# vribeiro1/artspeech

Hardware: AMD Instinct MI355X
Metric: articulator-frames/sec (fwd+bwd) (higher is better)
Workload: dtype f32

## Files before the change

### artspeech_amd/csrc/gru.hip

```cpp
#include <cstdlib>

#include <type_traits>

#include <hip/hip_ext.h>

#include "as_common.h"
#include "gemm_internal.h"

namespace {

typedef float f32x2 __attribute__((ext_vector_type(2)));

template <int LPU>
__device__ __forceinline__ float unit_sum(float v) {
    v += __int_as_float(__builtin_amdgcn_update_dpp(0, __float_as_int(v), 0xB1, 0xF, 0xF, true));
    if (LPU == 4) v += __int_as_float(__builtin_amdgcn_update_dpp(0, __float_as_int(v), 0x4E, 0xF, 0xF, true));
    return v;
}

constexpr int AHEAD = 2;

template <int H, int LPU, bool TRAIN, bool TOK>
__global__ __launch_bounds__(LPU * H) void gru_fwd_kernel(const float* __restrict__ gi, const int64_t* __restrict__ tokens,
                                                          long tok_stride, const float* __restrict__ w_hh,
                                                          const float* __restrict__ b_hh, const int* __restrict__ lengths,
                                                          int T, float* __restrict__ y, float* __restrict__ gates, int nd, int V) {
    constexpr int CW = 4 * LPU;
    constexpr int NC = H / CW;
    constexpr int NT = LPU * H;
    __shared__ __attribute__((aligned(16))) float hbuf[3][H];
    extern __shared__ int tok_s[];
    const int b = blockIdx.x, dir = blockIdx.y;
    const int tid = threadIdx.x, j = tid / LPU, q = tid % LPU;
    const int len = lengths[b];

    f32x2 w[3][NC * 2];
    {
        const float* wd = w_hh + (long)dir * 3 * H * H;
#pragma unroll
        for (int g = 0; g < 3; ++g)
#pragma unroll
            for (int c = 0; c < NC; ++c) {
                const float4 v = *reinterpret_cast<const float4*>(wd + (long)(g * H + j) * H + CW * c + 4 * q);
                w[g][2 * c] = f32x2{v.x, v.y};
                w[g][2 * c + 1] = f32x2{v.z, v.w};
            }
    }
    const float bq_r = b_hh[dir * 3 * H + j] * (1.0f / LPU), bq_z = b_hh[dir * 3 * H + H + j] * (1.0f / LPU),
                bq_n = b_hh[dir * 3 * H + 2 * H + j] * (1.0f / LPU);

    for (long i = (long)len * H + tid; i < (long)T * H; i += NT)
        y[((long)b * T + i / H) * nd * H + dir * H + (i % H)] = 0.f;
    if (tid < H) hbuf[0][tid] = 0.f;
    if (TOK)
        for (int t = tid; t < len; t += NT) {
            const int64_t v = tokens[(long)b * tok_stride + t];
            tok_s[t] = (int)(V > 0 ? min(max(v, (int64_t)0), (int64_t)V - 1) : v) * (nd * 3 * H * 4);
        }
    __syncthreads();
    if (len <= 0) return;

    const int t0 = dir ? len - 1 : 0;
    const int dt = dir ? -1 : 1;
    const unsigned ys = (unsigned)nd * H * 4u, gs = (unsigned)nd * 4u * H * 4u, is = (unsigned)nd * 3u * H * 4u;
    const unsigned yo = (unsigned)(dir * H + j) * 4u;
    const unsigned go = (unsigned)(dir * 4 * H + j + (LPU == 4 ? q * H : q * H)) * 4u;
    const unsigned io = (unsigned)(dir * 3 * H + j) * 4u;
    const char* gi_c = reinterpret_cast<const char*>(gi);
    char* y_c = reinterpret_cast<char*>(y);
    char* g_c = reinterpret_cast<char*>(gates);
    const int m0 = q == 0 ? -1 : 0, m1 = q == 1 ? -1 : 0, m2 = q == 2 ? -1 : 0, m3 = q == 3 ? -1 : 0;

    float h = 0.f;
    struct Gi { float r, z, n; };
    auto load_step = [&](int u) {
        const int uc = u < len ? u : len - 1;
        const int tu = t0 + uc * dt;
        const unsigned ro = (TOK ? (unsigned)tok_s[tu] : (unsigned)(b * T + tu) * is) + io;
        const float* p = reinterpret_cast<const float*>(gi_c + ro);
        return Gi{p[0], p[H], p[2 * H]};
    };
    auto step = [&](auto curc, int s, const Gi& ci, Gi& fill) {
        const int cur = curc, nxt = (cur + 1) % 3;
        const unsigned fr = (unsigned)(b * T + t0 + s * dt);
        fill = load_step(s + AHEAD);
        const float4* hp = reinterpret_cast<const float4*>(hbuf[cur]);
        f32x2 ar = {bq_r, 0.f}, az = {bq_z, 0.f}, an = {bq_n, 0.f};
#pragma unroll
        for (int c0 = 0; c0 < NC; c0 += 8) {
            float4 hv[8];
#pragma unroll
            for (int u = 0; u < 8; ++u)
                if (c0 + u < NC) hv[u] = hp[LPU * (c0 + u) + q];
            __builtin_amdgcn_sched_barrier(0);
#pragma unroll
            for (int u = 0; u < 8; ++u)
                if (c0 + u < NC) {
                    const int c = c0 + u;
                    const f32x2 lo = {hv[u].x, hv[u].y}, hi = {hv[u].z, hv[u].w};
                    ar = __builtin_elementwise_fma(w[0][2 * c], lo, ar);
                    az = __builtin_elementwise_fma(w[1][2 * c], lo, az);
                    an = __builtin_elementwise_fma(w[2][2 * c], lo, an);
                    ar = __builtin_elementwise_fma(w[0][2 * c + 1], hi, ar);
                    az = __builtin_elementwise_fma(w[1][2 * c + 1], hi, az);
                    an = __builtin_elementwise_fma(w[2][2 * c + 1], hi, an);
                }
        }
        const float sr = unit_sum<LPU>(ar.x + ar.y), sz = unit_sum<LPU>(az.x + az.y), sn = unit_sum<LPU>(an.x + an.y);
        float r, z;
        if constexpr (LPU == 4) {
            const float pre = __int_as_float((__float_as_int(ci.r + sr) & m0) | (__float_as_int(ci.z + sz) & ~m0));
            const float sg = as_sigmoid(pre);
            r = __int_as_float(__builtin_amdgcn_update_dpp(0, __float_as_int(sg), 0x00, 0xF, 0xF, true));
            z = __int_as_float(__builtin_amdgcn_update_dpp(0, __float_as_int(sg), 0x55, 0xF, 0xF, true));
        } else {
            r = as_sigmoid(ci.r + sr);
            z = as_sigmoid(ci.z + sz);
        }
        const float hn = sn;
        const float n = as_tanh(ci.n + r * hn);
        const float hnew = (1.f - z) * n + z * h;
        h = hnew;
        hbuf[nxt][j] = hnew;
        *reinterpret_cast<float*>(y_c + (fr * ys + yo)) = hnew;
        if (TRAIN) {
            float* gp = reinterpret_cast<float*>(g_c + (fr * gs + go));
            if (LPU == 4) {
                const int m01 = m0 | m1;
                const int t1 = (__float_as_int(r) & m0) | (__float_as_int(z) & ~m0);
                const int t2 = (__float_as_int(n) & m2) | (__float_as_int(hn) & ~m2);
                gp[0] = __int_as_float((t1 & m01) | (t2 & ~m01));
            } else {
                const int ga = (__float_as_int(r) & m0) | (__float_as_int(z) & m1);
                const int gc = (__float_as_int(n) & m0) | (__float_as_int(hn) & m1);
                gp[0] = __int_as_float(ga);
                gp[2 * H] = __int_as_float(gc);
            }
        }
        __syncthreads();
    };
    constexpr std::integral_constant<int, 0> c0{};
    constexpr std::integral_constant<int, 1> c1{};
    constexpr std::integral_constant<int, 2> c2{};
    Gi a = load_step(0), bq = load_step(1), c;
    int s = 0;
    for (; s + 2 < len; s += 3) {
        step(c0, s, a, c);
        step(c1, s + 1, bq, a);
        step(c2, s + 2, c, bq);
    }
    if (s < len) step(c0, s, a, c);
    if (s + 1 < len) step(c1, s + 1, bq, a);
}

template <int H, bool TOK, int ND = 2>
__global__ __launch_bounds__(4 * H) void gru_bwd_row_kernel(const float* __restrict__ dy, const float* __restrict__ y,
                                                            const float* __restrict__ gates, const float* __restrict__ w_hh,
                                                            const int* __restrict__ lengths, int T, float* __restrict__ dgi,
                                                            float* __restrict__ dgh, unsigned long long* __restrict__ dbg,
                                                            const int64_t* __restrict__ tokens, long tok_stride, int V,
                                                            float* __restrict__ part) {
    constexpr int NT = 4 * H;
    extern __shared__ float tab[];
    constexpr int VL = 3 * H / 16;
    unsigned long long t_start = 0, r_start = 0;
    if (dbg != nullptr && threadIdx.x == 0) {
        t_start = __builtin_amdgcn_s_memtime();
        r_start = __builtin_amdgcn_s_memrealtime();
    }
    constexpr int VW = VL % 4 == 0 ? 4 : 2;
    constexpr int NCH = VL / VW;
    __shared__ __attribute__((aligned(16))) float gbuf[3][3 * H];
    const int b = blockIdx.x, dir = blockIdx.y;
    const int tid = threadIdx.x, row = tid >> 4, r = tid & 15;
    const int k0 = row * 4, k = k0 + (r & 3), pl = r >> 2;
    const int len = lengths[b];

    f32x2 wt[4][VL / 2];
    {
        const float* wd = w_hh + (long)dir * 3 * H * H;
#pragma unroll
        for (int c = 0; c < NCH; ++c)
#pragma unroll
            for (int pp = 0; pp < VW / 2; ++pp) {
                const int i = (c * 16 + r) * VW + 2 * pp;
                const float4 lo = *reinterpret_cast<const float4*>(wd + (long)i * H + k0);
                const float4 hi = *reinterpret_cast<const float4*>(wd + (long)(i + 1) * H + k0);
                auto pick = [](const float4& v, int u) { return u == 0 ? v.x : u == 1 ? v.y : u == 2 ? v.z : v.w; };
#pragma unroll
                for (int sl = 0; sl < 4; ++sl) wt[sl][c * (VW / 2) + pp] = f32x2{pick(lo, (sl + (r & 3)) & 3), pick(hi, (sl + (r & 3)) & 3)};
            }
    }
    for (long i = (long)len * 3 * H + tid; i < (long)T * 3 * H; i += NT) {
        const long t = i / (3 * H), c = i % (3 * H);
        const long o = (((long)b * T + t) * ND + dir) * 3 * H + c;
        if constexpr (!TOK) dgi[o] = 0.f;
        dgh[o] = 0.f;
    }
    float* part_wg = nullptr;
    if constexpr (TOK) {
        for (int i = tid; i < V * 3 * H; i += NT) tab[i] = 0.f;
        int* toff = reinterpret_cast<int*>(tab + (long)V * 3 * H + NT);
        for (int t = tid; t < len; t += NT) toff[t] = (int)min(max(tokens[(long)b * tok_stride + t], (int64_t)0), (int64_t)V - 1) * (3 * H);
        part_wg = part + (long)b * V * 6 * H + (long)dir * 3 * H;
        if (len <= 0) {
            for (int i = tid; i < V * 3 * H; i += NT) part_wg[(long)(i / (3 * H)) * 6 * H + i % (3 * H)] = 0.f;
            return;
        }
    } else {
        if (len <= 0) return;
    }

    const int t0 = dir ? 0 : len - 1;
    const int dt = dir ? 1 : -1;
    const char* g_c = reinterpret_cast<const char*>(gates);
    const char* y_c = reinterpret_cast<const char*>(y);
    const char* dy_c = reinterpret_cast<const char*>(dy);
    char* dgi_c = reinterpret_cast<char*>(dgi);
    char* dgh_c = reinterpret_cast<char*>(dgh);
    const unsigned gto = (unsigned)(dir * 4 * H + k) * 4u;
    const unsigned yo = (unsigned)(dir * H + k) * 4u;
    const int sel = pl < 2 ? pl : 2;
    const unsigned dgo = (unsigned)(dir * 3 * H + sel * H + k) * 4u;
    struct In { float r, z, n, hn, hprev, dyv; bool has_prev; };
    auto load = [&](long fr, bool has_prev) {
        In v;
        const unsigned f = (unsigned)fr;
        const float* gp = reinterpret_cast<const float*>(g_c + (f * (ND * 4u * H * 4u) + gto));
        v.r = gp[0]; v.z = gp[H]; v.n = gp[2 * H]; v.hn = gp[3 * H];
        v.hprev = *reinterpret_cast<const float*>(y_c + ((f + (unsigned)(has_prev ? dt : 0)) * (ND * H * 4u) + yo));
        v.has_prev = has_prev;
        v.dyv = *reinterpret_cast<const float*>(dy_c + (f * (ND * H * 4u) + yo));
        return v;
    };
    auto dpp_add = [](float acc, float v, auto ctrl) {
        return acc + __int_as_float(__builtin_amdgcn_update_dpp(0, __float_as_int(v), decltype(ctrl)::value, 0xF, 0xF, true));
    };
    const long fbase = (long)b * T + t0;
    float dh = 0.f;
    const int tmask = pl < 3 ? -1 : 0;
    float* tabk = pl < 3 ? tab + sel * H + k : tab + (long)V * 3 * H + tid;
    const int* toff = reinterpret_cast<const int*>(tab + (long)V * 3 * H + NT);
    int toff_cur = 0;
    if constexpr (TOK) {
        __syncthreads();
        toff_cur = toff[t0];
    }
    auto load_step = [&](int u) {
        const int uc = u < len ? u : len - 1;
        return load(fbase + (long)uc * dt, uc + 1 < len);
    };
    auto step = [&](auto bulk, auto curc, int s, const In& ci, In& fill) {
        constexpr bool BULK = decltype(bulk)::value;
        const int cur = curc;
        const long fr = fbase + (long)s * dt;
        if constexpr (BULK) fill = load(fbase + (long)(s + AHEAD) * dt, true);
        else fill = load_step(s + AHEAD);

        const float rg = ci.r, z = ci.z, n = ci.n, hn = ci.hn;
        const float omz = 1.f - z;
        const float c_n = omz * (1.f - n * n);
        const float c_hn = c_n * rg;
        const float c_r = c_hn * hn * (1.f - rg);
        const float c_z = (((BULK || ci.has_prev) ? ci.hprev : 0.f) - n) * z * omz;
        const float c_rz = pl == 0 ? c_r : c_z;
        const float c_vi = pl >= 2 ? c_n : c_rz;
        const float c_vh = pl >= 2 ? c_hn : c_rz;
        const float dht = dh + ci.dyv;
        const float vi = dht * c_vi;
        const float vh = dht * c_vh;
        gbuf[cur][sel * H + k] = vh;
        const unsigned dfo = (unsigned)fr * (ND * 3u * H * 4u) + dgo;
        if constexpr (!TOK) *reinterpret_cast<float*>(dgi_c + dfo) = vi;
        *reinterpret_cast<float*>(dgh_c + dfo) = vh;
        __syncthreads();

        f32x2 a[4] = {{0.f, 0.f}, {0.f, 0.f}, {0.f, 0.f}, {0.f, 0.f}};
        if constexpr (VW == 4) {
            const float4* gq = reinterpret_cast<const float4*>(gbuf[cur]);
            float4 gv[NCH];
#pragma unroll
            for (int c = 0; c < NCH; ++c) gv[c] = gq[c * 16 + r];
            float* tw = nullptr;
            float told = 0.f;
            int toff_nxt = 0;
            if constexpr (TOK) {
                tw = tabk + (toff_cur & tmask);
                told = *tw;
                toff_nxt = toff[t0 + (s + 1 < len ? s + 1 : s) * dt];
            }
            __builtin_amdgcn_sched_barrier(0);
#pragma unroll
            for (int c = 0; c < NCH; ++c) {
                const f32x2 lo = {gv[c].x, gv[c].y}, hi = {gv[c].z, gv[c].w};
#pragma unroll
                for (int kk = 0; kk < 4; ++kk) {
                    a[kk] = __builtin_elementwise_fma(wt[kk][2 * c], lo, a[kk]);
                    a[kk] = __builtin_elementwise_fma(wt[kk][2 * c + 1], hi, a[kk]);
                }
            }
            if constexpr (TOK) {
                __builtin_amdgcn_sched_barrier(0);
                *tw = told + vi;
                toff_cur = toff_nxt;
            }
        } else {
            const float2* gq = reinterpret_cast<const float2*>(gbuf[cur]);
            float2 gv[NCH];
#pragma unroll
            for (int c = 0; c < NCH; ++c) gv[c] = gq[c * 16 + r];
            __builtin_amdgcn_sched_barrier(0);
#pragma unroll
            for (int c = 0; c < NCH; ++c) {
                const f32x2 g2 = {gv[c].x, gv[c].y};
#pragma unroll
                for (int kk = 0; kk < 4; ++kk) a[kk] = __builtin_elementwise_fma(wt[kk][c], g2, a[kk]);
            }
            if constexpr (TOK) {
                tabk[toff_cur & tmask] += vi;
                toff_cur = toff[t0 + (s + 1 < len ? s + 1 : s) * dt];
            }
        }
        float acc = a[0].x + a[0].y;
        acc = dpp_add(acc, a[3].x + a[3].y, std::integral_constant<int, 0x39>{});
        acc = dpp_add(acc, a[2].x + a[2].y, std::integral_constant<int, 0x4E>{});
        acc = dpp_add(acc, a[1].x + a[1].y, std::integral_constant<int, 0x93>{});
        acc = dpp_add(acc, acc, std::integral_constant<int, 0x124>{});
        acc = dpp_add(acc, acc, std::integral_constant<int, 0x128>{});
        dh = dht * z + acc;
    };
    constexpr std::integral_constant<int, 0> c0{};
    constexpr std::integral_constant<int, 1> c1{};
    constexpr std::integral_constant<int, 2> c2{};
    In a = load_step(0), bq = load_step(1), c;
    int s = 0;
    constexpr std::true_type yes{};
    constexpr std::false_type no{};
    for (; s + 5 < len; s += 3) {
        step(yes, c0, s, a, c);
        step(yes, c1, s + 1, bq, a);
        step(yes, c2, s + 2, c, bq);
    }
    for (; s + 2 < len; s += 3) {
        step(no, c0, s, a, c);
        step(no, c1, s + 1, bq, a);
        step(no, c2, s + 2, c, bq);
    }
    if (s < len) step(no, c0, s, a, c);
    if (s + 1 < len) step(no, c1, s + 1, bq, a);
    if constexpr (TOK) {
        __syncthreads();
        for (int i = tid; i < V * 3 * H; i += NT) part_wg[(long)(i / (3 * H)) * 6 * H + i % (3 * H)] = tab[i];
    }
    if (dbg != nullptr && threadIdx.x == 0) {
        unsigned long long* d = dbg + 4L * (blockIdx.y * gridDim.x + blockIdx.x);
        d[0] = __builtin_amdgcn_s_memtime() - t_start;
        d[1] = __builtin_amdgcn_s_memrealtime() - r_start;
        d[2] = (unsigned long long)len;
        d[3] = r_start;
    }
}


constexpr int GEN_THREADS = 1024;

template <bool TRAIN, bool TOK>
__global__ __launch_bounds__(GEN_THREADS) void gru_fwd_generic_kernel(const float* __restrict__ gi, const int64_t* __restrict__ tokens,
                                                                     long tok_stride, const float* __restrict__ w_hh,
                                                                     const float* __restrict__ b_hh, const int* __restrict__ lengths,
                                                                     int T, int H, float* __restrict__ y, float* __restrict__ gates,
                                                                     int nd, int V) {
    extern __shared__ __attribute__((aligned(16))) float gsm[];
    const int b = blockIdx.x, dir = blockIdx.y, tid = threadIdx.x;
    const int q = tid & 3;
    const int len = lengths[b];
    for (long i = (long)len * H + tid; i < (long)T * H; i += GEN_THREADS)
        y[((long)b * T + i / H) * nd * H + dir * H + (i % H)] = 0.f;
    for (int j = tid; j < 2 * H; j += GEN_THREADS) gsm[j] = 0.f;
    __syncthreads();
    if (len <= 0) return;
    const float* wd = w_hh + (long)dir * 3 * H * H;
    const float* bd = b_hh + (long)dir * 3 * H;
    const int nch = H >> 2;
    for (int s = 0; s < len; ++s) {
        const int t = dir ? len - 1 - s : s;
        const long frame = (long)b * T + t;
        const float* hc = gsm + (s & 1) * H;
        float* hn_ = gsm + ((s & 1) ^ 1) * H;
        const float* gr;
        if (TOK) {
            int64_t v = tokens[(long)b * tok_stride + t];
            if (V > 0) v = v < 0 ? 0 : (v >= V ? V - 1 : v);
            gr = gi + (v * nd + dir) * 3L * H;
        } else {
            gr = gi + (frame * nd + dir) * 3L * H;
        }
        for (int j = tid >> 2; j < H; j += GEN_THREADS / 4) {
            const float4* wr = reinterpret_cast<const float4*>(wd + (long)j * H);
            const float4* wz = reinterpret_cast<const float4*>(wd + (long)(H + j) * H);
            const float4* wn = reinterpret_cast<const float4*>(wd + (long)(2 * H + j) * H);
            const float4* h4 = reinterpret_cast<const float4*>(hc);
            float sr = 0.f, sz = 0.f, sn = 0.f;
            for (int c0 = q; c0 < nch; c0 += 16) {
                float4 a[4], c[4], e[4], hv[4];
#pragma unroll
                for (int u = 0; u < 4; ++u) {
                    const int cc = c0 + 4 * u;
                    const int ci = cc < nch ? cc : nch - 1;
                    a[u] = wr[ci]; c[u] = wz[ci]; e[u] = wn[ci];
                    hv[u] = h4[ci];
                    if (cc >= nch) hv[u] = make_float4(0.f, 0.f, 0.f, 0.f);
                }
#pragma unroll
                for (int u = 0; u < 4; ++u) {
                    sr += a[u].x * hv[u].x + a[u].y * hv[u].y + a[u].z * hv[u].z + a[u].w * hv[u].w;
                    sz += c[u].x * hv[u].x + c[u].y * hv[u].y + c[u].z * hv[u].z + c[u].w * hv[u].w;
                    sn += e[u].x * hv[u].x + e[u].y * hv[u].y + e[u].z * hv[u].z + e[u].w * hv[u].w;
                }
            }
            sr = unit_sum<4>(sr) + bd[j];
            sz = unit_sum<4>(sz) + bd[H + j];
            sn = unit_sum<4>(sn) + bd[2 * H + j];
            const float r = as_sigmoid(gr[j] + sr);
            const float z = as_sigmoid(gr[H + j] + sz);
            const float n = as_tanh(gr[2 * H + j] + r * sn);
            const float hnew = (1.f - z) * n + z * hc[j];
            if (q == 0) {
                hn_[j] = hnew;
                y[(frame * nd + dir) * H + j] = hnew;
                if (TRAIN) {
                    float* gp = gates + (frame * nd + dir) * 4L * H + j;
                    gp[0] = r; gp[H] = z; gp[2 * H] = n; gp[3 * H] = sn;
                }
            }
        }
        __syncthreads();
    }
}

__global__ __launch_bounds__(GEN_THREADS) void gru_bwd_generic_kernel(const float* __restrict__ dy, const float* __restrict__ y,
                                                                     const float* __restrict__ gates, const float* __restrict__ w_hh,
                                                                     const int* __restrict__ lengths, int T, int H,
                                                                     float* __restrict__ dgi, float* __restrict__ dgh, int nd) {
    extern __shared__ __attribute__((aligned(16))) float gsm[];
    float* gb = gsm;
    float* dhb = gsm + 3 * H;
    float* dhz = gsm + 4 * H;
    float* part = gsm + 5 * H;
    const int b = blockIdx.x, dir = blockIdx.y, tid = threadIdx.x;
    const int len = lengths[b];
    for (long i = (long)len * 3 * H + tid; i < (long)T * 3 * H; i += GEN_THREADS) {
        const long t = i / (3 * H), c = i % (3 * H);
        const long o = (((long)b * T + t) * nd + dir) * 3 * H + c;
        dgi[o] = 0.f;
        dgh[o] = 0.f;
    }
    for (int j = tid; j < H; j += GEN_THREADS) dhb[j] = 0.f;
    __syncthreads();
    if (len <= 0) return;
    const float* wd = w_hh + (long)dir * 3 * H * H;
    const int dt = dir ? 1 : -1;
    const int kq = tid >> 8, kl = tid & 255;
    for (int s = 0; s < len; ++s) {
        const int t = dir ? s : len - 1 - s;
        const long frame = (long)b * T + t;
        const bool has_prev = s + 1 < len;
        for (int j = tid; j < H; j += GEN_THREADS) {
            const float* gp = gates + (frame * nd + dir) * 4L * H + j;
            const float r = gp[0], z = gp[H], n = gp[2 * H], hn = gp[3 * H];
            const float hprev = has_prev ? y[((frame + dt) * nd + dir) * H + j] : 0.f;
            const float dht = dhb[j] + dy[(frame * nd + dir) * H + j];
            const float dn = dht * (1.f - z);
            const float dz = dht * (hprev - n);
            const float dnt = dn * (1.f - n * n);
            const float g_r = dnt * hn * r * (1.f - r);
            const float g_z = dz * z * (1.f - z);
            const float g_hn = dnt * r;
            float* di = dgi + (frame * nd + dir) * 3L * H + j;
            float* dh = dgh + (frame * nd + dir) * 3L * H + j;
            di[0] = g_r; di[H] = g_z; di[2 * H] = dnt;
            dh[0] = g_r; dh[H] = g_z; dh[2 * H] = g_hn;
            gb[j] = g_r; gb[H + j] = g_z; gb[2 * H + j] = g_hn;
            dhz[j] = dht * z;
        }
        __syncthreads();
        for (int k0 = 0; k0 < H; k0 += 256) {
            const int k = k0 + kl;
            const int kc = k < H ? k : H - 1;
            float acc = 0.f;
            for (int i0 = kq; i0 < 3 * H; i0 += 32) {
                float wv[8], gv[8];
#pragma unroll
                for (int u = 0; u < 8; ++u) {
                    const int i = i0 + 4 * u;
                    const int ic = i < 3 * H ? i : 3 * H - 1;
                    wv[u] = wd[(long)ic * H + kc];
                    gv[u] = i < 3 * H ? gb[ic] : 0.f;
                }
#pragma unroll
                for (int u = 0; u < 8; ++u) acc += gv[u] * wv[u];
            }
            if (k < H) part[kq * H + k] = acc;
        }
        __syncthreads();
        for (int k = tid; k < H; k += GEN_THREADS) dhb[k] = dhz[k] + ((part[k] + part[H + k]) + (part[2 * H + k] + part[3 * H + k]));
        __syncthreads();
    }
}

constexpr int lpu_of(int) { return 4; }

}

constexpr size_t GRU_LDS_PAD = 144 * 1024, GRU_LDS_ATTR = 152 * 1024;
static size_t gru_lds_pad(int workgroups) {
    static const bool off = getenv("ARTSPEECH_GRU_SHARED_CUS") != nullptr;
    if (off) return 0;
    static const int cus = [] {
        int dev = 0, n = 0;
        if (hipGetDevice(&dev) != hipSuccess || hipDeviceGetAttribute(&n, hipDeviceAttributeMultiprocessorCount, dev) != hipSuccess) n = 0;
        return n;
    }();
    return workgroups * 2 <= cus ? GRU_LDS_PAD : 0;
}
template <typename K>
static bool gru_lds_attr(K kernel) {
    static const hipError_t e = hipFuncSetAttribute(reinterpret_cast<const void*>(kernel), hipFuncAttributeMaxDynamicSharedMemorySize, (int)GRU_LDS_ATTR);
    return e == hipSuccess;
}

static unsigned long long* g_gru_dbg = nullptr;
static unsigned g_gru_dbg_launch = 0;
constexpr int AS_GRU_TOK_LDS_MAX = 128 * 1024;
extern "C" void as_gru_debug_stamps(uint64_t* buf) { g_gru_dbg = (unsigned long long*)buf; g_gru_dbg_launch = 0; }

static int gru_fwd_launch(const float* gi, const int64_t* tokens, int64_t tok_stride, const float* w_hh, const float* b_hh,
                          const int32_t* lengths, int32_t B, int32_t T, int32_t H, float* y, float* gates, int nd, void* stream,
                          int V = 0) {
    AS_REQUIRE(gi && w_hh && b_hh && lengths && y, AS_ERR_BAD_ARG, "as_gru_fwd: null pointer");
    AS_REQUIRE(B > 0 && T > 0, AS_ERR_BAD_ARG, "as_gru_fwd: B=%d T=%d", B, T);
    AS_REQUIRE(!tokens || T <= 32768, AS_ERR_UNSUPPORTED, "as_gru_fwd: T=%d > 32768 with a token table", T);
    AS_REQUIRE((long)B * T * nd * 4 * H * 4 < (1L << 32), AS_ERR_UNSUPPORTED, "as_gru_fwd: B*T=%ld frames exceed the 32-bit offsets", (long)B * T);
    hipStream_t st = (hipStream_t)stream;
    dim3 grid(B, nd);
    const size_t pad = gru_lds_pad(B * nd);
    const size_t need = tokens ? (size_t)T * sizeof(int) : 0;
#define AS_GRU_LAUNCH(HH, TR, TK)                                                                                      \
    do {                                                                                                               \
        const size_t shm = pad > need && gru_lds_attr(gru_fwd_kernel<HH, lpu_of(HH), TR, TK>) ? pad : need;            \
        hipLaunchKernelGGL((gru_fwd_kernel<HH, lpu_of(HH), TR, TK>), grid, dim3(lpu_of(HH) * HH), shm, st, gi, tokens, \
                           (long)tok_stride, w_hh, b_hh, lengths, T, y, gates, nd, V);                                 \
    } while (0)
#define AS_GRU_FWD(HH)                                      \
    if (gates && tokens) AS_GRU_LAUNCH(HH, true, true);     \
    else if (gates) AS_GRU_LAUNCH(HH, true, false);         \
    else if (tokens) AS_GRU_LAUNCH(HH, false, true);        \
    else AS_GRU_LAUNCH(HH, false, false)
    switch (H) {
        case 32: AS_GRU_FWD(32); break;
        case 64: AS_GRU_FWD(64); break;
        case 128: AS_GRU_FWD(128); break;
        default: {
            const size_t gshm = (size_t)2 * H * sizeof(float);
            AS_REQUIRE(H > 0 && H % 4 == 0 && gshm <= 64 * 1024, AS_ERR_UNSUPPORTED, "as_gru_fwd: hidden size %d (a multiple of 4 up to 8192)", H);
#define AS_GRU_GEN(TR, TK) \
    hipLaunchKernelGGL((gru_fwd_generic_kernel<TR, TK>), grid, dim3(GEN_THREADS), gshm, st, gi, tokens, (long)tok_stride, w_hh, b_hh, lengths, T, H, y, gates, nd, V)
            if (gates && tokens) AS_GRU_GEN(true, true);
            else if (gates) AS_GRU_GEN(true, false);
            else if (tokens) AS_GRU_GEN(false, true);
            else AS_GRU_GEN(false, false);
#undef AS_GRU_GEN
        }
    }
#undef AS_GRU_FWD
#undef AS_GRU_LAUNCH
    AS_LAUNCH_CHECK("as_gru_fwd");
    return 0;
}

extern "C" int as_gru_bidir_fwd(const float* gi, const int64_t* tokens, int64_t tok_stride, const float* w_hh,
                                const float* b_hh, const int32_t* lengths, int32_t B, int32_t T, int32_t H, float* y,
                                float* gates, void* stream) {
    return gru_fwd_launch(gi, tokens, tok_stride, w_hh, b_hh, lengths, B, T, H, y, gates, 2, stream);
}

int as_gru_bidir_fwd_tokens(const float* table, const int64_t* tokens, int64_t tok_stride, int32_t V, const float* w_hh,
                            const float* b_hh, const int32_t* lengths, int32_t B, int32_t T, int32_t H, float* y, float* gates,
                            hipStream_t st) {
    return gru_fwd_launch(table, tokens, tok_stride, w_hh, b_hh, lengths, B, T, H, y, gates, 2, st, V);
}

extern "C" int as_gru_unidir_fwd(const float* gi, const float* w_hh, const float* b_hh, const int32_t* lengths, int32_t B,
                                 int32_t T, int32_t H, float* y, void* stream) {
    return gru_fwd_launch(gi, nullptr, 0, w_hh, b_hh, lengths, B, T, H, y, nullptr, 1, stream);
}

extern "C" int as_gru_unidir_fwd_gates(const float* gi, const float* w_hh, const float* b_hh, const int32_t* lengths, int32_t B,
                                       int32_t T, int32_t H, float* y, float* gates, void* stream) {
    AS_REQUIRE(gates, AS_ERR_BAD_ARG, "as_gru_unidir_fwd_gates: null pointer");
    return gru_fwd_launch(gi, nullptr, 0, w_hh, b_hh, lengths, B, T, H, y, gates, 1, stream);
}

static int gru_bwd_launch(const float* dy, const float* y, const float* gates, const float* w_hh, const int32_t* lengths,
                          int32_t B, int32_t T, int32_t H, float* dgi, float* dgh, const int64_t* tokens, int64_t tok_stride,
                          int32_t V, float* part, void* stream, int nd = 2) {
    AS_REQUIRE(dy && y && gates && w_hh && lengths && (dgi || tokens) && dgh, AS_ERR_BAD_ARG, "as_gru_bidir_bwd: null pointer");
    AS_REQUIRE(B > 0 && T > 0, AS_ERR_BAD_ARG, "as_gru_bidir_bwd: B=%d T=%d", B, T);
    AS_REQUIRE(!tokens || (part && V > 0 && tok_stride >= T && nd == 2), AS_ERR_BAD_ARG, "as_gru_bidir_bwd: token table arguments");
    AS_REQUIRE((long)B * T * nd * 4 * H * 4 < (1L << 32), AS_ERR_UNSUPPORTED, "as_gru_bidir_bwd: B*T=%ld frames exceed the 32-bit offsets", (long)B * T);
    hipStream_t st = (hipStream_t)stream;
    dim3 grid(B, nd);
    unsigned long long* dbg_now = g_gru_dbg ? g_gru_dbg + (size_t)(g_gru_dbg_launch++ & 1u) * 8u * (size_t)B : nullptr;
    hipEvent_t stop_ev = (H == 32 || H == 64 || H == 128) ? as_stop_event_take() : nullptr;
    const size_t pad = gru_lds_pad(B * nd);
    const size_t need = tokens ? ((size_t)V * 3 * H + 4 * H + T) * sizeof(float) : 0;
#define AS_GRU_BWD_ROW(HH, TK, ND)                                                                                     \
    do {                                                                                                                      \
        const bool big = gru_lds_attr(gru_bwd_row_kernel<HH, TK, ND>);                                                    \
        AS_REQUIRE(big || need <= 64 * 1024, AS_ERR_UNSUPPORTED, "as_gru_bidir_bwd: cannot reserve %zu bytes of LDS", need);   \
        const size_t shm = big && pad > need ? pad : need;                                                                    \
        if (stop_ev)                            \
            hipExtLaunchKernelGGL((gru_bwd_row_kernel<HH, TK, ND>), grid, dim3(4 * HH), (unsigned)shm, st, nullptr, stop_ev, 0, dy, \
                                  y, gates, w_hh, lengths, T, dgi, dgh, dbg_now, tokens, (long)tok_stride, V, part);          \
        else                                                                                                                  \
            hipLaunchKernelGGL((gru_bwd_row_kernel<HH, TK, ND>), grid, dim3(4 * HH), shm, st, dy, y, gates, w_hh,         \
                               lengths, T, dgi, dgh, dbg_now, tokens, (long)tok_stride, V, part);                             \
    } while (0)
#define AS_GRU_BWD(HH) \
    if (tokens) AS_GRU_BWD_ROW(HH, true, 2); else AS_GRU_BWD_ROW(HH, false, 2)
    if (nd == 1 && (H == 32 || H == 64 || H == 128)) {
        if (H == 32) AS_GRU_BWD_ROW(32, false, 1);
        else if (H == 64) AS_GRU_BWD_ROW(64, false, 1);
        else AS_GRU_BWD_ROW(128, false, 1);
    } else switch (H) {
        case 32: AS_GRU_BWD(32); break;
        case 64: AS_GRU_BWD(64); break;
        case 128: AS_GRU_BWD(128); break;
        default: {
            AS_REQUIRE(!tokens && dgi, AS_ERR_UNSUPPORTED, "as_gru_bidir_bwd: token sums need a hidden size in {32, 64, 128}");
            const size_t gshm = (size_t)9 * H * sizeof(float);
            AS_REQUIRE(H > 0 && H % 4 == 0 && gshm <= 64 * 1024, AS_ERR_UNSUPPORTED, "as_gru_bidir_bwd: hidden size %d (a multiple of 4 up to 1820)", H);
            hipLaunchKernelGGL(gru_bwd_generic_kernel, grid, dim3(GEN_THREADS), gshm, st, dy, y, gates, w_hh, lengths, T, H, dgi, dgh, nd);
        }
    }
#undef AS_GRU_BWD
#undef AS_GRU_BWD_ROW
    AS_LAUNCH_CHECK("as_gru_bidir_bwd");
    return 0;
}

extern "C" int as_gru_bidir_bwd(const float* dy, const float* y, const float* gates, const float* w_hh,
                                const int32_t* lengths, int32_t B, int32_t T, int32_t H, float* dgi, float* dgh,
                                void* stream) {
    AS_REQUIRE(dgi, AS_ERR_BAD_ARG, "as_gru_bidir_bwd: null pointer");
    return gru_bwd_launch(dy, y, gates, w_hh, lengths, B, T, H, dgi, dgh, nullptr, 0, 0, nullptr, stream);
}

bool as_gru_bwd_tokens_fits(int32_t V, int32_t H, int32_t T) {
    return (H == 32 || H == 64 || H == 128) && ((long)V * 3 * H + 4 * H + T) * (long)sizeof(float) <= AS_GRU_TOK_LDS_MAX;
}
int as_gru_bidir_bwd_tokens(const float* dy, const float* y, const float* gates, const float* w_hh, const int32_t* lengths,
                            int32_t B, int32_t T, int32_t H, float* dgh, const int64_t* tokens, int64_t tok_stride, int32_t V,
                            float* part, hipStream_t st) {
    if (!tokens || !as_gru_bwd_tokens_fits(V, H, T)) return 0;
    const int rc = gru_bwd_launch(dy, y, gates, w_hh, lengths, B, T, H, nullptr, dgh, tokens, tok_stride, V, part, st);
    return rc == 0 ? 1 : rc;
}

extern "C" int as_gru_unidir_bwd(const float* dy, const float* y, const float* gates, const float* w_hh, const int32_t* lengths,
                                 int32_t B, int32_t T, int32_t H, float* dgi, float* dgh, void* stream) {
    AS_REQUIRE(dgi, AS_ERR_BAD_ARG, "as_gru_unidir_bwd: null pointer");
    return gru_bwd_launch(dy, y, gates, w_hh, lengths, B, T, H, dgi, dgh, nullptr, 0, 0, nullptr, stream, 1);
}
```

Before: 6.426 million.

## Software-pipeline GRU backward gate coefficients and batch token-table scatter updates

In the backward row kernel, the gate-derivative coefficients for the next step are computed one step early, overlapping the recurrent matvec. Token-table gradient scatters are deferred and flushed every three steps using int4-packed offsets stored in step order, with duplicate-token handling. In the forward kernel, the token row offset is prefetched one step ahead so the dependent load chain is shortened. This adds register pressure and more complex LDS offset layout and tail handling.

Measured after the change: 6.436 million, median of 5. No clear change (+0.1%).

```diff
diff --git a/artspeech_amd/csrc/gru.hip b/artspeech_amd/csrc/gru.hip
--- a/artspeech_amd/csrc/gru.hip
+++ b/artspeech_amd/csrc/gru.hip
@@ -80,10 +80,17 @@
         const float* p = reinterpret_cast<const float*>(gi_c + ro);
         return Gi{p[0], p[H], p[2 * H]};
     };
+    auto tok_row = [&](int u) { return tok_s[t0 + (u < len ? u : len - 1) * dt]; };
+    int tok_ro = TOK ? tok_row(AHEAD) : 0;
     auto step = [&](auto curc, int s, const Gi& ci, Gi& fill) {
         const int cur = curc, nxt = (cur + 1) % 3;
         const unsigned fr = (unsigned)(b * T + t0 + s * dt);
-        fill = load_step(s + AHEAD);
+        if constexpr (TOK) {
+            const float* p = reinterpret_cast<const float*>(gi_c + ((unsigned)tok_ro + io));
+            fill = Gi{p[0], p[H], p[2 * H]};
+        } else {
+            fill = load_step(s + AHEAD);
+        }
         const float4* hp = reinterpret_cast<const float4*>(hbuf[cur]);
         f32x2 ar = {bq_r, 0.f}, az = {bq_z, 0.f}, an = {bq_n, 0.f};
 #pragma unroll
@@ -92,6 +99,7 @@
 #pragma unroll
             for (int u = 0; u < 8; ++u)
                 if (c0 + u < NC) hv[u] = hp[LPU * (c0 + u) + q];
+            if (TOK && c0 == 0) tok_ro = tok_row(s + AHEAD + 1);
             __builtin_amdgcn_sched_barrier(0);
 #pragma unroll
             for (int u = 0; u < 8; ++u)
@@ -161,7 +169,7 @@
                                                             const int64_t* __restrict__ tokens, long tok_stride, int V,
                                                             float* __restrict__ part) {
     constexpr int NT = 4 * H;
-    extern __shared__ float tab[];
+    extern __shared__ __attribute__((aligned(16))) float tab[];
     constexpr int VL = 3 * H / 16;
     unsigned long long t_start = 0, r_start = 0;
     if (dbg != nullptr && threadIdx.x == 0) {
@@ -197,11 +205,14 @@
         if constexpr (!TOK) dgi[o] = 0.f;
         dgh[o] = 0.f;
     }
+    const int t0 = dir ? 0 : len - 1;
+    const int dt = dir ? 1 : -1;
     float* part_wg = nullptr;
     if constexpr (TOK) {
         for (int i = tid; i < V * 3 * H; i += NT) tab[i] = 0.f;
         int* toff = reinterpret_cast<int*>(tab + (long)V * 3 * H + NT);
-        for (int t = tid; t < len; t += NT) toff[t] = (int)min(max(tokens[(long)b * tok_stride + t], (int64_t)0), (int64_t)V - 1) * (3 * H);
+        for (int u = tid; u < len; u += NT)
+            toff[(u / 3) * 4 + u % 3] = (int)min(max(tokens[(long)b * tok_stride + t0 + u * dt], (int64_t)0), (int64_t)V - 1) * (3 * H);
         part_wg = part + (long)b * V * 6 * H + (long)dir * 3 * H;
         if (len <= 0) {
             for (int i = tid; i < V * 3 * H; i += NT) part_wg[(long)(i / (3 * H)) * 6 * H + i % (3 * H)] = 0.f;
@@ -211,8 +222,6 @@
         if (len <= 0) return;
     }
 
-    const int t0 = dir ? 0 : len - 1;
-    const int dt = dir ? 1 : -1;
     const char* g_c = reinterpret_cast<const char*>(gates);
     const char* y_c = reinterpret_cast<const char*>(y);
     const char* dy_c = reinterpret_cast<const char*>(dy);
@@ -240,56 +249,75 @@
     float dh = 0.f;
     const int tmask = pl < 3 ? -1 : 0;
     float* tabk = pl < 3 ? tab + sel * H + k : tab + (long)V * 3 * H + tid;
-    const int* toff = reinterpret_cast<const int*>(tab + (long)V * 3 * H + NT);
-    int toff_cur = 0;
-    if constexpr (TOK) {
-        __syncthreads();
-        toff_cur = toff[t0];
-    }
+    const int4* toff4 = reinterpret_cast<const int4*>(tab + (long)V * 3 * H + NT);
+    if constexpr (TOK) __syncthreads();
     auto load_step = [&](int u) {
         const int uc = u < len ? u : len - 1;
         return load(fbase + (long)uc * dt, uc + 1 < len);
     };
-    auto step = [&](auto bulk, auto curc, int s, const In& ci, In& fill) {
-        constexpr bool BULK = decltype(bulk)::value;
-        const int cur = curc;
-        const long fr = fbase + (long)s * dt;
-        if constexpr (BULK) fill = load(fbase + (long)(s + AHEAD) * dt, true);
-        else fill = load_step(s + AHEAD);
-
+    struct Cf { float vi, vh, z, dyv; };
+    auto coef = [&](bool has_prev, const In& ci) {
         const float rg = ci.r, z = ci.z, n = ci.n, hn = ci.hn;
         const float omz = 1.f - z;
-        const float c_n = omz * (1.f - n * n);
+        const float c_n = omz * __builtin_fmaf(-n, n, 1.f);
         const float c_hn = c_n * rg;
         const float c_r = c_hn * hn * (1.f - rg);
-        const float c_z = (((BULK || ci.has_prev) ? ci.hprev : 0.f) - n) * z * omz;
+        const float c_z = ((has_prev ? ci.hprev : 0.f) - n) * z * omz;
         const float c_rz = pl == 0 ? c_r : c_z;
-        const float c_vi = pl >= 2 ? c_n : c_rz;
-        const float c_vh = pl >= 2 ? c_hn : c_rz;
-        const float dht = dh + ci.dyv;
-        const float vi = dht * c_vi;
-        const float vh = dht * c_vh;
-        gbuf[cur][sel * H + k] = vh;
+        return Cf{pl >= 2 ? c_n : c_rz, pl >= 2 ? c_hn : c_rz, z, ci.dyv};
+    };
+    constexpr int LA = 3;
+    float vq[3] = {0.f, 0.f, 0.f}, cq[3] = {0.f, 0.f, 0.f};
+    int4 og = {0, 0, 0, 0};
+    Cf kq[3];
+    auto step = [&](auto bulk, auto posc, auto flush, int s, const In& nx, In& fill) {
+        constexpr bool BULK = decltype(bulk)::value;
+        constexpr int POS = decltype(posc)::value;
+        constexpr bool FLUSH = TOK && decltype(flush)::value;
+        const long fr = fbase + (long)s * dt;
+        if constexpr (BULK) fill = load(fbase + (long)(s + LA) * dt, true);
+        else fill = load_step(s + LA);
+
+        const Cf& kc = kq[POS];
+        const float dht = dh + kc.dyv;
+        const float vi = dht * kc.vi;
+        const float vh = dht * kc.vh;
+        gbuf[POS][sel * H + k] = vh;
         const unsigned dfo = (unsigned)fr * (ND * 3u * H * 4u) + dgo;
-        if constexpr (!TOK) *reinterpret_cast<float*>(dgi_c + dfo) = vi;
+        if constexpr (!TOK) {
+            *reinterpret_cast<float*>(dgi_c + dfo) = vi;
+        } else {
+            vq[POS] = dht;
+            cq[POS] = kc.vi;
+        }
         *reinterpret_cast<float*>(dgh_c + dfo) = vh;
         __syncthreads();
 
         f32x2 a[4] = {{0.f, 0.f}, {0.f, 0.f}, {0.f, 0.f}, {0.f, 0.f}};
+        float4 gv[VW == 4 ? NCH : 1];
+        float2 gv2[VW == 2 ? NCH : 1];
         if constexpr (VW == 4) {
-            const float4* gq = reinterpret_cast<const float4*>(gbuf[cur]);
-            float4 gv[NCH];
+            const float4* gq = reinterpret_cast<const float4*>(gbuf[POS]);
 #pragma unroll
             for (int c = 0; c < NCH; ++c) gv[c] = gq[c * 16 + r];
-            float* tw = nullptr;
-            float told = 0.f;
-            int toff_nxt = 0;
-            if constexpr (TOK) {
-                tw = tabk + (toff_cur & tmask);
-                told = *tw;
-                toff_nxt = toff[t0 + (s + 1 < len ? s + 1 : s) * dt];
-            }
-            __builtin_amdgcn_sched_barrier(0);
+        } else {
+            const float2* gq = reinterpret_cast<const float2*>(gbuf[POS]);
+#pragma unroll
+            for (int c = 0; c < NCH; ++c) gv2[c] = gq[c * 16 + r];
+        }
+        float t0w = 0.f, t1w = 0.f, t2w = 0.f;
+        if constexpr (TOK && POS == 0) og = toff4[s / 3];
+        if constexpr (FLUSH) {
+            t0w = tabk[og.x & tmask];
+            t1w = tabk[og.y & tmask];
+            t2w = tabk[og.z & tmask];
+        }
+        __builtin_amdgcn_sched_barrier(0);
+        Cf& kn = kq[(POS + 1) % 3];
+        kn = coef(BULK || nx.has_prev, nx);
+        asm volatile("" : "+v"(kn.vi), "+v"(kn.vh));
+        __builtin_amdgcn_sched_barrier(0);
+        if constexpr (VW == 4) {
 #pragma unroll
             for (int c = 0; c < NCH; ++c) {
                 const f32x2 lo = {gv[c].x, gv[c].y}, hi = {gv[c].z, gv[c].w};
@@ -299,27 +327,22 @@
                     a[kk] = __builtin_elementwise_fma(wt[kk][2 * c + 1], hi, a[kk]);
                 }
             }
-            if constexpr (TOK) {
-                __builtin_amdgcn_sched_barrier(0);
-                *tw = told + vi;
-                toff_cur = toff_nxt;
-            }
         } else {
-            const float2* gq = reinterpret_cast<const float2*>(gbuf[cur]);
-            float2 gv[NCH];
-#pragma unroll
-            for (int c = 0; c < NCH; ++c) gv[c] = gq[c * 16 + r];
-            __builtin_amdgcn_sched_barrier(0);
 #pragma unroll
             for (int c = 0; c < NCH; ++c) {
-                const f32x2 g2 = {gv[c].x, gv[c].y};
+                const f32x2 g2 = {gv2[c].x, gv2[c].y};
 #pragma unroll
                 for (int kk = 0; kk < 4; ++kk) a[kk] = __builtin_elementwise_fma(wt[kk][c], g2, a[kk]);
             }
-            if constexpr (TOK) {
-                tabk[toff_cur & tmask] += vi;
-                toff_cur = toff[t0 + (s + 1 < len ? s + 1 : s) * dt];
-            }
+        }
+        if constexpr (FLUSH) {
+            __builtin_amdgcn_sched_barrier(0);
+            const float s0 = __builtin_fmaf(vq[0], cq[0], t0w);
+            const float s1 = __builtin_fmaf(vq[1], cq[1], og.y == og.x ? s0 : t1w);
+            const float s2 = __builtin_fmaf(vq[2], cq[2], og.z == og.y ? s1 : og.z == og.x ? s0 : t2w);
+            tabk[og.x & tmask] = s0;
+            tabk[og.y & tmask] = s1;
+            tabk[og.z & tmask] = s2;
         }
         float acc = a[0].x + a[0].y;
         acc = dpp_add(acc, a[3].x + a[3].y, std::integral_constant<int, 0x39>{});
@@ -327,28 +350,31 @@
         acc = dpp_add(acc, a[1].x + a[1].y, std::integral_constant<int, 0x93>{});
         acc = dpp_add(acc, acc, std::integral_constant<int, 0x124>{});
         acc = dpp_add(acc, acc, std::integral_constant<int, 0x128>{});
-        dh = dht * z + acc;
+        dh = dht * kc.z + acc;
     };
-    constexpr std::integral_constant<int, 0> c0{};
-    constexpr std::integral_constant<int, 1> c1{};
-    constexpr std::integral_constant<int, 2> c2{};
-    In a = load_step(0), bq = load_step(1), c;
-    int s = 0;
+    constexpr std::integral_constant<int, 0> p0{};
+    constexpr std::integral_constant<int, 1> p1{};
+    constexpr std::integral_constant<int, 2> p2{};
     constexpr std::true_type yes{};
     constexpr std::false_type no{};
-    for (; s + 5 < len; s += 3) {
-        step(yes, c0, s, a, c);
-        step(yes, c1, s + 1, bq, a);
-        step(yes, c2, s + 2, c, bq);
+    In a = load_step(0), bq = load_step(1), c = load_step(2);
+    kq[0] = coef(a.has_prev, a);
+    int s = 0;
+    for (; s + 2 + LA + 1 < len; s += 3) {
+        step(yes, p0, no, s, bq, a);
+        step(yes, p1, no, s + 1, c, bq);
+        step(yes, p2, yes, s + 2, a, c);
     }
     for (; s + 2 < len; s += 3) {
-        step(no, c0, s, a, c);
-        step(no, c1, s + 1, bq, a);
-        step(no, c2, s + 2, c, bq);
-    }
-    if (s < len) step(no, c0, s, a, c);
-    if (s + 1 < len) step(no, c1, s + 1, bq, a);
+        step(no, p0, no, s, bq, a);
+        step(no, p1, no, s + 1, c, bq);
+        step(no, p2, yes, s + 2, a, c);
+    }
+    if (s < len) step(no, p0, no, s, bq, a);
+    if (s + 1 < len) step(no, p1, no, s + 1, c, bq);
     if constexpr (TOK) {
+        if (s < len) tabk[og.x & tmask] = __builtin_fmaf(vq[0], cq[0], tabk[og.x & tmask]);
+        if (s + 1 < len) tabk[og.y & tmask] = __builtin_fmaf(vq[1], cq[1], tabk[og.y & tmask]);
         __syncthreads();
         for (int i = tid; i < V * 3 * H; i += NT) part_wg[(long)(i / (3 * H)) * 6 * H + i % (3 * H)] = tab[i];
     }
@@ -532,6 +558,7 @@
 static unsigned long long* g_gru_dbg = nullptr;
 static unsigned g_gru_dbg_launch = 0;
 constexpr int AS_GRU_TOK_LDS_MAX = 128 * 1024;
+static long gru_bwd_tok_lds(long V, long H, long T) { return (V * 3 * H + 4 * H + (T + 2) / 3 * 4) * (long)sizeof(float); }
 extern "C" void as_gru_debug_stamps(uint64_t* buf) { g_gru_dbg = (unsigned long long*)buf; g_gru_dbg_launch = 0; }
 
 static int gru_fwd_launch(const float* gi, const int64_t* tokens, int64_t tok_stride, const float* w_hh, const float* b_hh,
@@ -613,7 +640,7 @@
     unsigned long long* dbg_now = g_gru_dbg ? g_gru_dbg + (size_t)(g_gru_dbg_launch++ & 1u) * 8u * (size_t)B : nullptr;
     hipEvent_t stop_ev = (H == 32 || H == 64 || H == 128) ? as_stop_event_take() : nullptr;
     const size_t pad = gru_lds_pad(B * nd);
-    const size_t need = tokens ? ((size_t)V * 3 * H + 4 * H + T) * sizeof(float) : 0;
+    const size_t need = tokens ? (size_t)gru_bwd_tok_lds(V, H, T) : 0;
 #define AS_GRU_BWD_ROW(HH, TK, ND)                                                                                     \
     do {                                                                                                                      \
         const bool big = gru_lds_attr(gru_bwd_row_kernel<HH, TK, ND>);                                                    \
@@ -657,7 +684,7 @@
 }
 
 bool as_gru_bwd_tokens_fits(int32_t V, int32_t H, int32_t T) {
-    return (H == 32 || H == 64 || H == 128) && ((long)V * 3 * H + 4 * H + T) * (long)sizeof(float) <= AS_GRU_TOK_LDS_MAX;
+    return (H == 32 || H == 64 || H == 128) && gru_bwd_tok_lds(V, H, T) <= AS_GRU_TOK_LDS_MAX;
 }
 int as_gru_bidir_bwd_tokens(const float* dy, const float* y, const float* gates, const float* w_hh, const int32_t* lengths,
                             int32_t B, int32_t T, int32_t H, float* dgh, const int64_t* tokens, int64_t tok_stride, int32_t V,
```
